# sharwarimarathe/GossipProtocol

Hardware: AMD Instinct MI355X
Metric: node-updates/sec (whole node) + achieved HBM GB/s %, imp3D push-sum 1e9 nodes (higher is better)
Workload: dtype f64; 1 GPU; push-sum rounds, Imp3D lattice, n=1000000000 (P=1000000000), steady state (all nodes active), seed 1; num_nodes=1000000000, population=1000000000, topology=Imp3D, algorithm=push-sum, parallelism=slab1, transport=none (one GPU), launcher=single process, activation_preroll_rounds=72

## Files before the change

### gossipprotocol_amd/csrc/gp_device.hpp

```cpp
#pragma once

#include <hip/hip_runtime.h>
#include <stdint.h>

#define GP_HD __host__ __device__ __forceinline__

namespace gp {

enum Topology : int { LINE = 0, FULL = 1, GRID3D = 2, IMP3D = 3 };
enum Algorithm : int { GOSSIP = 0, PUSHSUM = 1 };
enum Stream : uint32_t { S_TOPO = 0, S_START = 1, S_GOSSIP = 2, S_PUSHSUM = 3, S_INJECT = 4 };

constexpr uint8_t DIR_MASK = 7, DIR_NONE = 7, DIR_RANDOM = 6;
constexpr uint8_t B_ACTIVE = 8, B_CONV = 16;
constexpr int CNT_SHIFT = 5;
constexpr uint32_t GOSSIP_DONE = 11;

GP_HD uint32_t xor3(uint32_t a, uint32_t b, uint32_t k) {
#if defined(__HIP_DEVICE_COMPILE__)
    uint32_t r;
    asm("v_bitop3_b32 %0, %1, %2, %3 bitop3:0x96" : "=v"(r) : "v"(a), "v"(b), "s"(k));
    return r;
#else
    return a ^ b ^ k;
#endif
}

GP_HD void philox2(uint32_t node, uint32_t round, uint32_t stream, uint32_t k0, uint32_t k1,
                   uint32_t& x, uint32_t& y) {
    uint32_t c0 = node, c1 = round, c2 = stream, c3 = 0;
#if defined(__HIP_DEVICE_COMPILE__)
    asm volatile("" : "+s"(k0), "+s"(k1));
#endif
#pragma unroll
    for (int r = 0; r < 10; ++r) {
        if (r) {
            k0 += 0x9E3779B9u;
            k1 += 0xBB67AE85u;
        }
        const uint64_t p0 = (uint64_t)0xD2511F53u * c0;
        const uint64_t p1 = (uint64_t)0xCD9E8D57u * c2;
        const uint32_t n0 = xor3((uint32_t)(p1 >> 32), c1, k0);
        const uint32_t n2 = xor3((uint32_t)(p0 >> 32), c3, k1);
        c1 = (uint32_t)p1;
        c3 = (uint32_t)p0;
        c0 = n0;
        c2 = n2;
    }
    x = c0;
    y = c1;
}

template <int N>
GP_HD void philox2_batch(const uint32_t (&node)[N], uint32_t round, uint32_t stream, uint32_t k0, uint32_t k1,
                         uint32_t (&x)[N], uint32_t (&y)[N]) {
    uint32_t c0[N], c1[N], c2[N], c3[N];
#pragma unroll
    for (int i = 0; i < N; ++i) {
        c0[i] = node[i];
        c1[i] = round;
        c2[i] = stream;
        c3[i] = 0;
    }
#if defined(__HIP_DEVICE_COMPILE__)
    asm volatile("" : "+s"(k0), "+s"(k1));
#endif
#pragma unroll
    for (int r = 0; r < 10; ++r) {
        if (r) {
            k0 += 0x9E3779B9u;
            k1 += 0xBB67AE85u;
        }
#pragma unroll
        for (int i = 0; i < N; ++i) {
            const uint64_t p0 = (uint64_t)0xD2511F53u * c0[i];
            const uint64_t p1 = (uint64_t)0xCD9E8D57u * c2[i];
            const uint32_t n0 = xor3((uint32_t)(p1 >> 32), c1[i], k0);
            const uint32_t n2 = xor3((uint32_t)(p0 >> 32), c3[i], k1);
            c1[i] = (uint32_t)p1;
            c3[i] = (uint32_t)p0;
            c0[i] = n0;
            c2[i] = n2;
        }
    }
#pragma unroll
    for (int i = 0; i < N; ++i) {
        x[i] = c0[i];
        y[i] = c1[i];
    }
}

GP_HD uint32_t uniform_from(uint32_t x, uint32_t y, uint32_t m) {
    const uint64_t lo = (uint64_t)x * m;
    const uint64_t hi = (uint64_t)y * m + (lo >> 32);
    return (uint32_t)(hi >> 32);
}

GP_HD uint32_t uniform(uint32_t k0, uint32_t k1, uint32_t stream, uint32_t node, uint32_t round,
                       uint32_t m) {
    uint32_t x, y;
    philox2(node, round, stream, k0, k1, x, y);
    return uniform_from(x, y, m);
}

GP_HD bool ratio_moved(double s, double w, double s2, double w2) {
    const double a = s * w2;
    const double b = __builtin_fma(s2, w, -a);
    const double m = w * w2;
    if (m >= 0x1p-900 && (s == 0.0 || a >= 0x1p-900) && __builtin_fabs(b) > 0x1p-18 * m) return true;
    return __builtin_fabs(s2 / w2 - s / w) > 1e-10;
}

struct FastDiv {
    uint32_t d;
    uint32_t magic;
    uint32_t shift;
    uint32_t mode;
};

inline FastDiv make_fastdiv(uint32_t d) {
    FastDiv f{d, 0, 0, 0};
    if (d == 0) return f;
    const uint32_t l = 31u - (uint32_t)__builtin_clz(d);
    if ((d & (d - 1)) == 0) {
        f.shift = l;
        f.mode = 0;
        return f;
    }
    const uint64_t num = 1ull << (32 + l);
    uint32_t proposed = (uint32_t)(num / d);
    const uint32_t rem = (uint32_t)(num % d);
    const uint32_t e = d - rem;
    if (e < (1u << l)) {
        f.shift = l;
        f.mode = 1;
    } else {
        proposed += proposed;
        const uint32_t twice_rem = rem + rem;
        if (twice_rem >= d || twice_rem < rem) proposed += 1;
        f.shift = l;
        f.mode = 2;
    }
    f.magic = 1u + proposed;
    return f;
}

GP_HD uint32_t mulhi32(uint32_t a, uint32_t b) { return (uint32_t)(((uint64_t)a * b) >> 32); }

GP_HD uint32_t fastdiv(uint32_t n, const FastDiv& f) {
    if (f.mode == 0) return n >> f.shift;
    const uint32_t q = mulhi32(f.magic, n);
    if (f.mode == 1) return q >> f.shift;
    const uint32_t t = ((n - q) >> 1) + q;
    return t >> f.shift;
}

struct Geom {
    uint32_t P;
    uint32_t T;
    uint32_t g, g2;
    FastDiv div_g, div_g2;
};

template <int TOPO>
GP_HD uint32_t present_mask(uint32_t j, const Geom& G) {
    if (TOPO == LINE) return (j > 0 ? 1u : 0u) | (j + 1 < G.P ? 2u : 0u);
    const uint32_t x = fastdiv(j, G.div_g2);
    const uint32_t rem = j - x * G.g2;
    const uint32_t y = fastdiv(rem, G.div_g);
    const uint32_t z = rem - y * G.g;
    const uint32_t gm = G.g - 1;
    return (x > 0 ? 1u : 0u) | (x < gm ? 2u : 0u) | (y < gm ? 4u : 0u) | (y > 0 ? 8u : 0u) |
           (z < gm ? 16u : 0u) | (z > 0 ? 32u : 0u);
}

template <int TOPO>
GP_HD uint32_t nbr(uint32_t j, uint32_t d, const Geom& G) {
    if (TOPO == LINE) return d == 0 ? j - 1 : j + 1;
    switch (d) {
        case 0: return j - G.g2;
        case 1: return j + G.g2;
        case 2: return j + G.g;
        case 3: return j - G.g;
        case 4: return j + 1;
        default: return j - 1;
    }
}

GP_HD uint32_t popc6(uint32_t m) {
#if defined(__HIP_DEVICE_COMPILE__)
    return (uint32_t)__popc(m);
#else
    return (uint32_t)__builtin_popcount(m);
#endif
}

GP_HD uint32_t slot_to_dir(uint32_t mask, uint32_t k) {
#pragma unroll
    for (uint32_t d = 0; d < 6; ++d) {
        if (mask & (1u << d)) {
            if (k == 0) return d;
            --k;
        }
    }
    return DIR_RANDOM;
}

GP_HD uint32_t slot_to_dir_fast(uint32_t mask, uint32_t k) {
    if (mask == 63u) return k < 6u ? k : (uint32_t)DIR_RANDOM;
    return slot_to_dir(mask, k);
}

GP_HD uint32_t mask_xyz(uint32_t x, uint32_t y, uint32_t z, uint32_t gm) {
    return (x > 0 ? 1u : 0u) | (x < gm ? 2u : 0u) | (y < gm ? 4u : 0u) | (y > 0 ? 8u : 0u) | (z < gm ? 16u : 0u) |
           (z > 0 ? 32u : 0u);
}

GP_HD uint32_t full_target(uint32_t i, uint32_t k) { return k < i ? k : k + 1; }

}
```

### gossipprotocol_amd/csrc/gp_ps_tile.hip

```cpp
#include <type_traits>

#include "gp_tile.hpp"

namespace gp {
#ifdef GP_TILE_WIDE
namespace wide {
#endif

constexpr int PRIO = 1;

namespace {

template <bool REMOTE>
struct PsSlots {
    static constexpr bool SNDPF = !REMOTE;
    static constexpr int SLOTS = SNDPF ? TILE + TILE / 8 : TILE + TILE / 8 + TILE / 16;
    static constexpr int FU = (SLOTS + TPB - 1) / TPB;
};

template <bool REMOTE>
struct TileLdsP {
    static constexpr int SLOTS = PsSlots<REMOTE>::SLOTS, SLOT_FU = PsSlots<REMOTE>::FU;
    uint32_t rows[W_ROWS + DMA_SLACK];
    uint32_t xm[W_PLANE + DMA_SLACK];
    uint32_t xp[W_PLANE + DMA_SLACK];
    uint32_t ind[TILE / 8 + DMA_SLACK];
    unsigned long long bits[SLOT_FU * (TPB / 64) + 1];
    double2 msg[SLOTS];
    uint32_t out[TILE / 4];
    uint32_t red[2][TPB / 64];
    uint32_t qn[2];
    double2 zb[TPB / 64][NPT][2];
};

}

template <int TOPO, bool REMOTE>
__device__ __forceinline__ void ps_tiles(const RoundArgs& a, uint32_t r, TileLdsP<REMOTE>& L, uint32_t* snd,
                                         bool all_active, uint32_t& alerts, uint32_t& newly, bool& tiny) {
    const double2* __restrict__ swc = a.swc;
    double2* __restrict__ swn = a.swn;
    const uint64_t* __restrict__ rbc = a.rbc;
    const uint32_t* __restrict__ in_src = a.in_src;
    const bool packed = a.in_srcd != nullptr;
    const uint32_t* __restrict__ srcp = packed ? a.in_srcd : in_src;
    const Geom G = a.G;
    const uint32_t H = TOPO == LINE ? 1u : G.g;
    constexpr int FU = PsSlots<REMOTE>::FU;
    const uint32_t cap = min((uint32_t)PsSlots<REMOTE>::SLOTS, a.stage_cap);
    const uint32_t lane = threadIdx.x & 63u, wv = threadIdx.x >> 6;

    uint32_t pf_tile = 0xFFFFFFFFu, pf_lo = 0, pf_hi = 0;
    uint32_t snd_tile = 0xFFFFFFFFu, snd_off = 0;
    constexpr bool SNDPF = PsSlots<REMOTE>::SNDPF;
    uint32_t raw[FU];
#pragma unroll
    for (int m = 0; m < FU; ++m) raw[m] = 0u;
    TileWalk tw(a);
    const bool dyn = tw.mode == 3;
    uint32_t it = 0;
    if (dyn) {
        if (blockIdx.x == 0 && threadIdx.x < 8) a.tq_next[threadIdx.x * TQ_STRIDE] = 0u;
        if (threadIdx.x == 0) L.qn[0] = atomicAdd(tw.qc, 1u);
        __syncthreads();
        tw.t = __builtin_amdgcn_readfirstlane(L.qn[0]);
        ++it;
    }
    for (uint32_t victim = 0;;) {
    while (tw.t < tw.end) {
        uint32_t ti;
        uint32_t claim = 0;
        if (dyn && threadIdx.x == 0) claim = atomicAdd(tw.qc, 1u);
        if (!tw.tile(ti)) {
            if (dyn) {
                if (threadIdx.x == 0) L.qn[it & 1] = claim;
                __syncthreads();
                tw.t = __builtin_amdgcn_readfirstlane(L.qn[it & 1]);
                ++it;
            } else {
                tw.t += tw.step;
            }
            continue;
        }
        const uint32_t T = (a.lo / TILE + ti) * TILE;
        const uint32_t j0 = max(a.lo, T);
        const uint32_t j1 = min(a.lo + a.nloc, T + TILE);
        const bool have_pf = pf_tile == ti;
        uint32_t e_lo = 0, e_hi = 0;
        if (TOPO == IMP3D) {
            if (have_pf) {
                e_lo = pf_lo;
                e_hi = pf_hi;
            } else {
                e_lo = ld_const(a.in_off + j0);
                e_hi = ld_const(a.in_off + j1);
            }
        }
        const uint32_t cnt = e_hi - e_lo;
        const bool staged = cnt <= cap;
        if (TOPO == IMP3D && !dyn) {
            TileWalk nw = tw;
            nw.t += nw.step;
            uint32_t nti;
            pf_tile = 0xFFFFFFFFu;
            if (nw.t < nw.end && nw.tile(nti)) {
                const uint32_t nT = (a.lo / TILE + nti) * TILE;
                pf_lo = ld_const(a.in_off + max(a.lo, nT));
                pf_hi = ld_const(a.in_off + min(a.lo + a.nloc, nT + TILE));
                pf_tile = nti;
            }
        }
        if constexpr (TOPO == IMP3D) {
            if (staged) {
                if (SNDPF && snd_tile == ti) {
                    uint32_t ts = threadIdx.x;
                    asm volatile("" : "+v"(ts));
#pragma unroll
                    for (int m = 0; m < FU; ++m) {
                        const uint32_t q = ts + m * TPB;
                        raw[m] = q < cnt ? snd[snd_off + q] : 0u;
                    }
                } else {
#pragma unroll
                    for (int m = 0; m < FU; ++m) {
                        const uint32_t q = threadIdx.x + m * TPB;
                        raw[m] = q < cnt ? __builtin_nontemporal_load(srcp + e_lo + q) : 0u;
                    }
                }
                uint32_t rkv[REMOTE ? FU : 1];
                if constexpr (REMOTE) {
#pragma unroll
                    for (int m = 0; m < FU; ++m) {
                        const uint32_t q = threadIdx.x + m * TPB;
                        rkv[m] = q < cnt ? __builtin_nontemporal_load(a.rk + e_lo + q) : 0u;
                    }
                }
                uint32_t isrc[FU];
                bool sent[FU], pick[FU];
#pragma unroll
                for (int m = 0; m < FU; ++m) isrc[m] = packed ? raw[m] & 0x3FFFFFFFu : raw[m];
                if (all_active) {
                    constexpr int F0 = FU < NPT ? FU : NPT;
                    uint32_t x[FU], y[FU];
                    {
                        uint32_t n0[F0], x0[F0], y0[F0];
#pragma unroll
                        for (int m = 0; m < F0; ++m) n0[m] = isrc[m];
                        philox2_batch<F0>(n0, r, S_PUSHSUM, a.k0, a.k1, x0, y0);
#pragma unroll
                        for (int m = 0; m < F0; ++m) {
                            x[m] = x0[m];
                            y[m] = y0[m];
                        }
                    }
#pragma unroll
                    for (int m = F0; m < FU; ++m) {
                        x[m] = y[m] = 0u;
                        if (cnt > (uint32_t)(m * TPB) + (__builtin_amdgcn_readfirstlane(threadIdx.x) & ~63u)) {
                            uint32_t n1[1] = {isrc[m]}, x1[1], y1[1];
                            philox2_batch<1>(n1, r, S_PUSHSUM, a.k0, a.k1, x1, y1);
                            x[m] = x1[0];
                            y[m] = y1[0];
                        }
                    }
#pragma unroll
                    for (int m = 0; m < FU; ++m) {
                        const uint32_t q = threadIdx.x + m * TPB;
                        const uint32_t di = packed ? (raw[m] >> 30) + 4u : popc6(present_mask<IMP3D>(isrc[m], G)) + 1u;
                        sent[m] = pick[m] = q < cnt && uniform_from(x[m], y[m], di) == di - 1u;
                    }
                } else {
                    uint32_t x[FU], y[FU];
                    philox2_batch<FU>(isrc, r, S_PUSHSUM, a.k0, a.k1, x, y);
                    bool lpick[FU];
#pragma unroll
                    for (int m = 0; m < FU; ++m) {
                        const uint32_t q = threadIdx.x + m * TPB;
                        const uint32_t i = isrc[m];
                        const uint32_t di = packed ? (raw[m] >> 30) + 4u : popc6(present_mask<IMP3D>(i, G)) + 1u;
                        pick[m] = q < cnt && uniform_from(x[m], y[m], di) == di - 1u;
                        lpick[m] = pick[m] && (!REMOTE || i - a.lo < a.nloc);
                    }
                    unsigned long long wbits[FU];
#pragma unroll
                    for (int m = 0; m < FU; ++m) wbits[m] = rbc[lpick[m] ? (isrc[m] >> 6) - (a.lo >> 6) : 0u];
#pragma unroll
                    for (int m = 0; m < FU; ++m) asm volatile("" : "+v"(wbits[m])::"memory");
#pragma unroll
                    for (int m = 0; m < FU; ++m) wbits[m] = lpick[m] ? wbits[m] : 0ull;
#pragma unroll
                    for (int m = 0; m < FU; ++m) sent[m] = (wbits[m] >> (isrc[m] & 63)) & 1ull;
                }
                uint32_t ridx[REMOTE ? FU : 1];
                if constexpr (REMOTE) {
                    uint2 hm[FU];
                    uint32_t hb[FU];
#pragma unroll
                    for (int m = 0; m < FU; ++m) {
                        const bool cand = pick[m] && isrc[m] - a.lo >= a.nloc;
                        const XHdr* hp = a.xhdr + (cand ? rkv[m] >> 6 : 0u);
                        hm[m] = *reinterpret_cast<const uint2*>(&hp->mask);
                        hb[m] = hp->base;
                    }
#pragma unroll
                    for (int m = 0; m < FU; ++m) asm volatile("" : "+v"(hm[m].x), "+v"(hm[m].y), "+v"(hb[m])::"memory");
#pragma unroll
                    for (int m = 0; m < FU; ++m) {
                        ridx[m] = 0u;
                        if (pick[m] && isrc[m] - a.lo >= a.nloc) {
                            const unsigned long long mk = ((unsigned long long)hm[m].y << 32) | hm[m].x;
                            const uint32_t bit = rkv[m] & 63u;
                            sent[m] = (mk >> bit) & 1ull;
                            ridx[m] = min(hb[m] + (uint32_t)__popcll(mk & ((1ull << bit) - 1ull)), a.xnv - 1u);
                        }
                    }
                }
                __builtin_amdgcn_s_setprio(PRIO);
#pragma unroll
                for (int m = 0; m < FU; ++m) {
                    const unsigned long long bal = __ballot(sent[m]);
                    if (lane == 0) L.bits[m * (TPB / 64) + wv] = bal;
                    if (sent[m]) {
                        const double2* src;
                        if constexpr (REMOTE) {
                            uint32_t xi = ridx[m];
                            asm volatile("" : "+v"(xi));
                            src = isrc[m] - a.lo >= a.nloc ? a.xvals + xi : swc + isrc[m];
                        } else {
                            src = swc + isrc[m];
                        }
                        __builtin_amdgcn_global_load_lds((gvoid_t*)src, (lvoid_t*)(L.msg + (m * TPB + wv * 64)), 16,
                                                         0, DMA_ONCE);
                    }
                }
                if (threadIdx.x == 0) {
                    unsigned long long z = 0ull;
                    asm volatile("" : "+v"(z));
                    L.bits[FU * (TPB / 64)] = z;
                }
            }
        }
        double2 own[NPT];
        const uint32_t b_rows = dma_stage_bytes(L.rows, a.nbc, (int64_t)j0 - H, (int64_t)j1 + H, a.ext_lo, a.ext_hi);
        uint32_t b_xm = 0, b_xp = 0;
        if (TOPO != LINE) {
            b_xm = dma_stage_bytes(L.xm, a.nbc, (int64_t)j0 - G.g2, (int64_t)j1 - G.g2, a.ext_lo, a.ext_hi);
            b_xp = dma_stage_bytes(L.xp, a.nbc, (int64_t)j0 + G.g2, (int64_t)j1 + G.g2, a.ext_lo, a.ext_hi);
        }
        {
            uint32_t zt = threadIdx.x;
            asm volatile("" : "+v"(zt));
            const uint32_t zl = zt & 63u, zw = zt >> 6;
            if (zl < 2u * NPT) {
                int64_t jn = (int64_t)T + (int64_t)((zl >> 1) * TPB + zw * 64u) + ((zl & 1u) ? 64 : -1);
                if (jn < (int64_t)a.ext_lo) jn = a.ext_lo;
                if (jn > (int64_t)a.ext_hi) jn = a.ext_hi;
                __builtin_amdgcn_global_load_lds((gvoid_t*)(swc + jn), (lvoid_t*)&L.zb[zw][0][0], 16, 0, 0);
            }
        }
        if (TOPO == IMP3D) {
            const uint8_t* ip = a.ind4 + T / 2;
            asm volatile("" : "+s"(ip));
            uint32_t nt = threadIdx.x;
            asm volatile("" : "+v"(nt));
            if (nt < (uint32_t)(TILE / 32))
                __builtin_amdgcn_global_load_lds((gvoid_t*)(ip + nt * 16u), (lvoid_t*)L.ind, 16, 0, DMA_ONCE);
        }
        if (dyn && threadIdx.x == 0) L.qn[it & 1] = claim;
        __builtin_amdgcn_s_setprio(0);
        __syncthreads();
        uint32_t cinc = 0;
        bool wide = false;
        if (TOPO == IMP3D) {
            const uint2 w2 = reinterpret_cast<const uint2*>(L.ind)[lane];
            auto nsum = [](uint32_t w) { return (((w & 0x0F0F0F0Fu) + ((w >> 4) & 0x0F0F0F0Fu)) * 0x01010101u) >> 24; };
            auto has15 = [](uint32_t w) { return (w & (w >> 1) & (w >> 2) & (w >> 3) & 0x11111111u) != 0u; };
            uint32_t incl = nsum(w2.x) + nsum(w2.y);
            wide = __ballot(has15(w2.x) || has15(w2.y)) != 0ull;
#pragma unroll
            for (int o = 1; o < 64; o <<= 1) {
                const uint32_t t = __shfl_up(incl, o, 64);
                if (lane >= (uint32_t)o) incl += t;
            }
            const uint32_t ex = __shfl_up(incl, 1, 64);
            cinc = lane == 0 ? 0u : ex;
        }
        uint32_t t_next = tw.t + tw.step;
        if (dyn) {
            t_next = __builtin_amdgcn_readfirstlane(L.qn[it & 1]);
            ++it;
            if (TOPO == IMP3D) {
                TileWalk nw = tw;
                nw.t = t_next;
                uint32_t nti;
                pf_tile = 0xFFFFFFFFu;
                if (nw.t < nw.end && nw.tile(nti)) {
                    const uint32_t nT = (a.lo / TILE + nti) * TILE;
                    pf_lo = ld_const(a.in_off + max(a.lo, nT));
                    pf_hi = ld_const(a.in_off + min(a.lo + a.nloc, nT + TILE));
                    pf_tile = nti;
                }
            }
        }

        bool full = j0 == T && j1 == T + TILE && (TOPO != IMP3D || (staged && !wide));
#ifdef GP_EXPERIMENTS
        if (a.no_full) full = false;
#endif
        auto tile_body = [&](auto full_c, auto shadow_c) {
        constexpr bool FULL = decltype(full_c)::value;
        constexpr bool SHADOW = decltype(shadow_c)::value;
        uint32_t tid = threadIdx.x;
        asm volatile("" : "+v"(tid));
        const uint32_t lane = tid & 63u, wv = tid >> 6;
        uint32_t pend[(NPT + 1) / 2];
#pragma unroll
        for (int k = 0; k < (NPT + 1) / 2; ++k) pend[k] = 0u;
        {
            const uint32_t wbase = __builtin_amdgcn_readfirstlane(tid & ~63u);
            uint32_t wcx = 0, wcy = 0, wcz = 0;
            if (TOPO != LINE) {
                const uint32_t jw = T + wbase;
                wcx = fastdiv(jw, G.div_g2);
                const uint32_t rem = jw - wcx * G.g2;
                wcy = fastdiv(rem, G.div_g);
                wcz = rem - wcy * G.g;
            }
            constexpr uint32_t NDG = TOPO == LINE ? 0u : 4u;
            auto decide = [&](const int k, uint32_t& gst, uint32_t& epre) {
                epre = 0u;
                uint32_t edeg = 0u;
                if (TOPO == IMP3D) {
                    const uint32_t jl = k * TPB + tid;
                    const uint32_t d = (lds_byte(L.ind, jl >> 1) >> ((jl & 1u) * 4u)) & 15u;
                    uint32_t ex = mbcnt64(__ballot(d & 1u)) + 2u * mbcnt64(__ballot(d & 2u));
                    if (__ballot(d >= 4u)) ex += 4u * mbcnt64(__ballot(d & 4u)) + 8u * mbcnt64(__ballot(d & 8u));
                    const int wvu = __builtin_amdgcn_readfirstlane((int)wv);
                    epre = (uint32_t)__builtin_amdgcn_readlane((int)cinc, 16 * k + 4 * wvu) + ex;
                    edeg = d;
                }
                const uint32_t j = T + k * TPB + tid;
                if (TOPO != LINE && k > 0) {
                    wcz += TPB;
                    if (wcz >= G.g) {
                        const uint32_t q = fastdiv(wcz, G.div_g);
                        wcz -= q * G.g;
                        wcy += q;
                        if (wcy >= G.g) {
                            const uint32_t q2 = fastdiv(wcy, G.div_g);
                            wcy -= q2 * G.g;
                            wcx += q2;
                        }
                    }
                }
                const uint32_t jr = j - b_rows;
                const uint32_t gbv = lds_byte(L.rows, jr);
                uint32_t mask;
                if (TOPO == LINE) {
                    mask = present_mask<TOPO>(j, G);
                } else {
                    const uint32_t gm = G.g - 1u;
                    const bool interior = wcz >= 1u && wcz + 64u < gm && wcy >= 1u && wcy < gm && wcx >= 1u && wcx < gm;
                    mask = interior ? 63u : present_mask<TOPO>(j, G);
                }
                uint32_t from = 0;
                if (TOPO == LINE) {
                    from |= ((mask & 1u) && (lds_byte(L.rows, (mask & 1u) ? jr - 1 : jr) & DIR_MASK) == 1u) ? 1u : 0u;
                    from |= ((mask & 2u) && (lds_byte(L.rows, (mask & 2u) ? jr + 1 : jr) & DIR_MASK) == 0u) ? 2u : 0u;
                } else {
                    const uint32_t bxm = lds_byte(L.xm, (mask & 1u) ? j - G.g2 - b_xm : 0u);
                    const uint32_t bxp = lds_byte(L.xp, (mask & 2u) ? j + G.g2 - b_xp : 0u);
                    const uint32_t byp = lds_byte(L.rows, (mask & 4u) ? jr + G.g : jr);
                    const uint32_t bym = lds_byte(L.rows, (mask & 8u) ? jr - G.g : jr);
                    uint32_t bzp, bzm;
                    if constexpr (FULL) {
                        const uint32_t be = lds_byte(L.rows, lane == 63u ? jr + 1u : max(jr, 1u) - 1u);
                        bzp = (uint32_t)__builtin_amdgcn_mov_dpp((int)gbv, 0x130, 0xF, 0xF, true);
                        bzm = (uint32_t)__builtin_amdgcn_mov_dpp((int)gbv, 0x138, 0xF, 0xF, true);
                        if (lane == 63u) bzp = be;
                        if (lane == 0u) bzm = be;
                    } else {
                        bzp = lds_byte(L.rows, (mask & 16u) ? jr + 1 : jr);
                        bzm = lds_byte(L.rows, (mask & 32u) ? jr - 1 : jr);
                    }
                    from =((bxm & DIR_MASK) == 1u ? 1u : 0u) | ((bxp & DIR_MASK) == 0u ? 2u : 0u) |
                           ((byp & DIR_MASK) == 3u ? 4u : 0u) | ((bym & DIR_MASK) == 2u ? 8u : 0u) |
                           ((bzp & DIR_MASK) == 5u ? 16u : 0u) | ((bzm & DIR_MASK) == 4u ? 32u : 0u);
                    from &= mask;
                }
                if (!FULL && !(j >= j0 && j < j1)) from = 0u;
                gst = gbv | (mask << 8) | (from << 14) | (edeg << 20);
            };
            constexpr bool AHEAD = SHADOW;
            uint32_t gst_n = 0u, epre_n = 0u;
            if (AHEAD) {
                __builtin_amdgcn_s_setprio(PRIO);
                decide(0, gst_n, epre_n);
            }
#pragma unroll
            for (int k = 0; k < NPT; ++k) {
                __builtin_amdgcn_s_setprio(PRIO);
                uint32_t gst, epre;
                if (AHEAD) {
                    gst = gst_n;
                    epre = epre_n;
                } else {
                    decide(k, gst, epre);
                }
                const uint32_t jl = k * TPB + tid;
                const uint32_t j = T + jl;
                double2 m[NDG > 0 ? NDG : 1];
                {
                    const uint32_t from = (gst >> 14) & 63u;
                    own[k] = swc[FULL ? j : min(max(j, j0), j1 - 1u)];
#pragma unroll
                    for (uint32_t d = 0; d < NDG; ++d)
                        m[d] = ld_sw(swc + ((from >> d) & 1u ? nbr<TOPO>(j, d, G) : a.ext_hi));
                }
                __builtin_amdgcn_s_setprio(0);
                if (SHADOW) __builtin_amdgcn_sched_barrier(0);
                {
                    const bool valid = FULL || (j >= j0 && j < j1);
                    uint32_t pwin = 0u, pqb = 0u;
                    if (TOPO == IMP3D && (FULL || (staged && !wide))) {
                        const uint32_t* bw = reinterpret_cast<const uint32_t*>(L.bits);
                        pqb = epre;
                        const uint32_t nd = gst >> 20;
                        pwin = __builtin_amdgcn_alignbit(bw[(pqb >> 5) + 1], bw[pqb >> 5], pqb & 31u) & ((1u << nd) - 1u);
                    }
                    if (SHADOW) {
                        uint32_t x, y;
                        philox2(j, r + 1, S_PUSHSUM, a.k0, a.k1, x, y);
                        const uint32_t mask = (gst >> 8) & 63u;
                        const uint32_t cand = slot_to_dir_fast(mask, uniform_from(x, y, popc6(mask) + (TOPO == IMP3D ? 1u : 0u)));
                        pend[k >> 1] |= cand << (16 * (k & 1));
                        if (AHEAD && k + 1 < NPT) decide(k + 1, gst_n, epre_n);
                        __builtin_amdgcn_sched_barrier(0);
                    }
                    double2 zP = make_double2(0.0, 0.0), zM = zP;
                    {
                        constexpr uint32_t dP = TOPO == LINE ? 1u : 4u, dM = TOPO == LINE ? 0u : 5u;
                        const uint32_t from = (gst >> 14) & 63u;
                        zP = dpp_double2<0x130>(own[k]);
                        zM = dpp_double2<0x138>(own[k]);
                        if (lane == 63u) zP = L.zb[wv][k][1];
                        if (lane == 0u) zM = L.zb[wv][k][0];
                        if (!((from >> dP) & 1u)) zP = make_double2(0.0, 0.0);
                        else if (!FULL && lane != 63u && j + 1u >= j1) zP = ld_sw(swc + j + 1);
                        if (!((from >> dM) & 1u)) zM = make_double2(0.0, 0.0);
                        else if (!FULL && lane != 0u && j <= j0) zM = ld_sw(swc + j - 1);
                    }
                    __builtin_amdgcn_s_waitcnt(vmcnt_enc(0));
                    if (valid) {
                        const uint32_t b = gst & 0xFFu, mask = (gst >> 8) & 63u, from = (gst >> 14) & 63u;
                        const uint32_t deg = popc6(mask) + (TOPO == IMP3D ? 1u : 0u);
                        bool active = (b & B_ACTIVE) != 0;
                        const double2 sv = own[k];

                        const bool halve = active && deg > 0;
                        const double hf = halve ? 0.5 : 1.0;
                        double acc_s = sv.x * hf;
                        double acc_w = sv.y * hf;
                        auto fold = [&](const double2 mi) {
                            acc_s = __builtin_fma(mi.x, 0.5, acc_s);
                            acc_w = __builtin_fma(mi.y, 0.5, acc_w);
                        };
                        tiny |= (sv.y < 0x1p-1020) | (sv.x != 0.0 && sv.x < 0x1p-1020);
                        bool recv = from != 0;
                        if (TOPO == LINE) {
                            fold(zM);
                            fold(zP);
                        } else {
#pragma unroll
                            for (uint32_t d = 0; d < NDG; ++d) fold(m[d]);
                            fold(zP);
                            fold(zM);
                        }
                        if (TOPO == IMP3D) {
                            uint32_t e_b = e_lo + epre, e_e = e_b + (gst >> 20);
                            if (!FULL && wide) {
                                e_b = a.in_off[j];
                                e_e = a.in_off[j + 1];
                            }
                            if (FULL || (staged && !wide)) {
                                uint32_t win = pwin;
                                while (win) {
                                    const uint32_t q = pqb + (uint32_t)__builtin_ctz(win);
                                    win &= win - 1u;
                                    fold(L.msg[q]);
                                    recv = true;
                                }
                            } else if (staged) {
                                const uint32_t* bw = reinterpret_cast<const uint32_t*>(L.bits);
                                const uint32_t qe = e_e - e_lo;
                                for (uint32_t q0 = e_b - e_lo; q0 < qe; q0 += 32u) {
                                    uint32_t win = __builtin_amdgcn_alignbit(bw[(q0 >> 5) + 1], bw[q0 >> 5], q0 & 31u);
                                    if (qe - q0 < 32u) win &= (1u << (qe - q0)) - 1u;
                                    while (win) {
                                        const uint32_t q = q0 + (uint32_t)__builtin_ctz(win);
                                        win &= win - 1u;
                                        fold(L.msg[q]);
                                        recv = true;
                                    }
                                }
                            } else {
                                for (uint32_t e = e_b; e < e_e; ++e) {
                                    const uint32_t i = in_src[e];
                                    bool sent;
                                    double2 mi = make_double2(0.0, 0.0);
                                    const bool rem = REMOTE && i - a.lo >= a.nloc;
                                    uint32_t xi = 0;
                                    if (rem) {
                                        const uint32_t k = a.rk[e];
                                        const XHdr h = a.xhdr[k >> 6];
                                        sent = (h.mask >> (k & 63u)) & 1ull;
                                        xi = min(h.base + (uint32_t)__popcll(h.mask & ((1ull << (k & 63u)) - 1ull)),
                                                 a.xnv - 1u);
                                    } else if (all_active) {
                                        const uint32_t di = popc6(present_mask<IMP3D>(i, G)) + 1u;
                                        sent = uniform(a.k0, a.k1, S_PUSHSUM, i, r, di) == di - 1u;
                                    } else {
                                        sent = (rbc[(i >> 6) - (a.lo >> 6)] >> (i & 63)) & 1ull;
                                    }
                                    if (sent) mi = rem ? a.xvals[xi] : ld_sw(swc + i);
                                    if (sent) {
                                        fold(mi);
                                        recv = true;
                                    }
                                }
                            }
                        }
                        uint32_t flags = b & (B_ACTIVE | B_CONV | (3u << CNT_SHIFT));
                        if (recv) {
                            if (!(b & B_CONV)) {
                                uint32_t cnt3 = (b >> CNT_SHIFT) & 3u;
                                cnt3 = ratio_moved(sv.x, sv.y, acc_s, acc_w) ? 0u : cnt3 + 1u;
                                flags = (flags & ~(3u << CNT_SHIFT)) | (cnt3 << CNT_SHIFT);
                                if (cnt3 == 3) {
                                    flags |= B_CONV;
                                    ++alerts;
                                }
                            }
                            if (!active) {
                                ++newly;
                                flags |= B_ACTIVE;
                                active = true;
                            }
                        }
                        if (SHADOW) {
                            pend[k >> 1] |= ((active && deg > 0 ? 0u : (uint32_t)DIR_NONE) | (flags & 0x78u)) << (16 * (k & 1));
                        } else {
                            pend[k >> 1] |= (mask | (active && deg > 0 ? 64u : 0u) | ((flags >> 3) << 7)) << (16 * (k & 1));
                        }
                        st_stream(swn + j, make_double2(acc_s, acc_w));
                    }
                }
                if (SNDPF && TOPO == IMP3D && k == 0) {
                    snd_tile = 0xFFFFFFFFu;
                    if (pf_tile != 0xFFFFFFFFu && pf_hi - pf_lo <= cap) {
                        snd_off = dma_stage_words(snd, srcp, pf_lo, pf_hi);
                        snd_tile = pf_tile;
                    }
                }
            }
        }
        {
            uint32_t node[NPT], x[NPT], y[NPT];
#pragma unroll
            for (int k = 0; k < NPT; ++k) node[k] = T + k * TPB + tid;
            if (!SHADOW) philox2_batch<NPT>(node, r + 1, S_PUSHSUM, a.k0, a.k1, x, y);
#pragma unroll
            for (int k = 0; k < NPT; ++k) {
                const uint32_t jl = k * TPB + tid;
                const bool valid = FULL || (node[k] >= j0 && node[k] < j1);
                const uint32_t pk = pend[k >> 1] >> (16 * (k & 1));
                uint32_t dir, nb;
                if (SHADOW) {
                    dir = pk & DIR_MASK;
                    nb = pk & 0x7Fu;
                } else {
                    const uint32_t mask = pk & 63u;
                    dir = DIR_NONE;
                    if (pk & 64u) dir = slot_to_dir_fast(mask, uniform_from(x[k], y[k], popc6(mask) + (TOPO == IMP3D ? 1u : 0u)));
                    nb = (((pk >> 7) & 15u) << 3) | dir;
                }
                if (valid) reinterpret_cast<uint8_t*>(L.out)[jl] = (uint8_t)nb;
                if (TOPO == IMP3D) {
                    const unsigned long long bits = __ballot(valid && dir == DIR_RANDOM);
                    if (lane == 0) {
                        const int64_t wi = (int64_t)((T + k * TPB + (tid & ~63u)) >> 6) - (int64_t)(a.lo >> 6);
                        if (wi >= 0) a.rbn[wi] = bits;
                    }
                }
            }
        }
        __syncthreads();
        for (uint32_t w = tid; w < (uint32_t)(TILE / 4); w += TPB) {
            const uint32_t jw = T + w * 4;
            if (FULL || (jw >= j0 && jw + 4 <= j1)) {
                st_stream(reinterpret_cast<uint32_t*>(a.nbn + T) + w, L.out[w]);
            } else {
                for (uint32_t b = 0; b < 4; ++b)
                    if (jw + b >= j0 && jw + b < j1) a.nbn[jw + b] = reinterpret_cast<const uint8_t*>(L.out)[w * 4 + b];
            }
        }
        };
#ifdef GP_EXPERIMENTS
        if (!a.slot_shadow) {
            if (full) tile_body(std::true_type{}, std::false_type{});
            else tile_body(std::false_type{}, std::false_type{});
        } else
#endif
        if (full) tile_body(std::true_type{}, std::true_type{});
        else tile_body(std::false_type{}, std::true_type{});
        tw.t = t_next;
    }
        if (!dyn || ++victim >= 8u) break;
        const uint32_t c = (blockIdx.x + victim) & 7u;
        tw.qc = a.tq + c * TQ_STRIDE;
        tw.wl = a.wt + a.wo[c];
        tw.end = a.wo[c + 1] - a.wo[c];
        if (threadIdx.x == 0) L.qn[it & 1] = atomicAdd(tw.qc, 1u);
        __syncthreads();
        tw.t = __builtin_amdgcn_readfirstlane(L.qn[it & 1]);
        ++it;
    }
}

__device__ __forceinline__ void block_counts(uint32_t (*red)[TPB / 64], uint32_t& x, uint32_t& y) {
    uint32_t tid = threadIdx.x;
    asm volatile("" : "+v"(tid));
    const uint32_t lane = tid & 63u, wv = tid >> 6;
#pragma unroll
    for (int o = 32; o > 0; o >>= 1) {
        x += __shfl_xor(x, o, 64);
        y += __shfl_xor(y, o, 64);
    }
    if (lane == 0) {
        red[0][wv] = x;
        red[1][wv] = y;
    }
    __syncthreads();
    if (threadIdx.x == 0) {
        x = 0;
        y = 0;
        for (int w = 0; w < TPB / 64; ++w) {
            x += red[0][w];
            y += red[1][w];
        }
    }
}

__device__ __forceinline__ void add_round_counts(Ctl* ctl, uint32_t x, uint32_t y) {
    unsigned long long d = 0;
    if (x) d += __hip_atomic_fetch_add(&ctl->round_alerts, (unsigned long long)x, __ATOMIC_RELAXED,
                                       __HIP_MEMORY_SCOPE_AGENT);
    if (y) d += __hip_atomic_fetch_add(&ctl->round_active, (unsigned long long)y, __ATOMIC_RELAXED,
                                       __HIP_MEMORY_SCOPE_AGENT);
    asm volatile("" ::"v"(d));
    __builtin_amdgcn_s_waitcnt(0);
}

template <int TOPO, bool REMOTE>
__global__ __launch_bounds__(TPB, GP_MINB) void k_ps_tile(RoundArgs a, uint32_t r) {
    __shared__ TileLdsP<REMOTE> L;
    __shared__ uint32_t snd[PsSlots<REMOTE>::SNDPF ? PsSlots<REMOTE>::SLOTS + DMA_SLACK : 1];
    Ctl* ctl = a.ctl;
    if (ld_agent(&ctl->done)) return;
    const bool all_active = ld_agent(&ctl->all_active) != 0;
    uint32_t alerts = 0, newly = 0;
    bool tiny = false;
    ps_tiles<TOPO, REMOTE>(a, r, L, snd, all_active, alerts, newly, tiny);
    if (__ballot(tiny) && (threadIdx.x & 63u) == 0) atomicOr(&ctl->tiny, 1u);
    block_counts(L.red, alerts, newly);
    if (threadIdx.x == 0) {
        if (a.fuse == 2) {
            block_done_close_sharded(ctl, a.G.P, a.G.T, r, alerts, newly);
        } else if (a.fuse) {
            add_round_counts(ctl, alerts, newly);
            block_done_close(ctl, a.G.P, a.G.T, r);
        } else {
            if (alerts) atomicAdd(&ctl->round_alerts, (unsigned long long)alerts);
            if (newly) atomicAdd(&ctl->round_active, (unsigned long long)newly);
        }
    }
}


using PsTileKernel = void (*)(RoundArgs, uint32_t);
static PsTileKernel ps_tile_kernel(int topo, bool remote) {
    if (topo == LINE) return k_ps_tile<LINE, false>;
    if (topo == GRID3D) return k_ps_tile<GRID3D, false>;
#ifndef GP_TILE_WIDE
    if (topo == IMP3D) return remote ? k_ps_tile<IMP3D, true> : k_ps_tile<IMP3D, false>;
#endif
    return nullptr;
}

int ps_tile_resident_blocks(int topo, bool remote, int device) {
    const PsTileKernel f = ps_tile_kernel(topo, remote);
    int per_cu = 0, cus = 0;
    if (!f) return 0;
    if (hipOccupancyMaxActiveBlocksPerMultiprocessor(&per_cu, reinterpret_cast<const void*>(f), TPB, 0) != hipSuccess)
        return 0;
    if (hipDeviceGetAttribute(&cus, hipDeviceAttributeMultiprocessorCount, device) != hipSuccess) return 0;
    return per_cu * cus;
}

hipError_t launch_ps_tile(const DevState& S, const RoundArgs& a, uint32_t round, int grid, hipStream_t st) {
    const PsTileKernel f = ps_tile_kernel(S.topo, S.rk != nullptr);
    if (!f || (S.topo == IMP3D && !S.ind4)) return hipErrorInvalidValue;
    hipLaunchKernelGGL(f, dim3(grid), dim3(TPB), 0, st, a, round);
    return hipGetLastError();
}

#ifdef GP_TILE_WIDE
}
#else
hipError_t launch_round_tile_region(const DevState& S, uint32_t round, uint32_t h, int grid, hipStream_t st) {
    if (S.alg != PUSHSUM || S.topo != IMP3D || !S.rk || !S.ind4 || !S.wtiles || S.tile_walk != 3 ||
        h >= S.rregions || (grid & 7))
        return hipErrorInvalidValue;
    RoundArgs a = make_round_args(S, round);
    for (int c = 0; c <= 8; ++c) a.wo[c] = S.woff[h][c];
    const uint64_t L = (uint64_t)round * S.rregions + h;
    a.tq = S.tq + (L & 1) * 8 * TQ_STRIDE;
    a.tq_next = S.tq + ((L + 1) & 1) * 8 * TQ_STRIDE;
    hipLaunchKernelGGL((k_ps_tile<IMP3D, true>), dim3(grid), dim3(TPB), 0, st, a, round);
    return hipGetLastError();
}
#endif
}
```

Before: 83.71 billion node-updates/s.

## Decode tile direction bytes four-per-lane with SWAR and redistribute via bpermute

For full interior tiles with four nodes per thread, each lane now reads one 32-bit word of direction bytes per neighbour plane and computes the six 'from' flags for four nodes at once using byte-parallel bit tricks. For Imp3D it also builds the per-node edge prefix offsets with a byte prefix sum plus DPP row scans. Each node's results are then fetched back to its owning lane with ds_bpermute. This is meant to replace per-node LDS byte loads and scalar decode in the decide step. It adds cross-lane permutes and more intricate index arithmetic, with risk of edge-case mistakes at tile borders.

```diff
diff --git a/gossipprotocol_amd/csrc/gp_device.hpp b/gossipprotocol_amd/csrc/gp_device.hpp
--- a/gossipprotocol_amd/csrc/gp_device.hpp
+++ b/gossipprotocol_amd/csrc/gp_device.hpp
@@ -216,6 +216,34 @@
            (z > 0 ? 32u : 0u);
 }
 
+
+GP_HD uint32_t byte_window(uint32_t lo, uint32_t hi, uint32_t ph) {
+#if defined(__HIP_DEVICE_COMPILE__)
+    return __builtin_amdgcn_alignbyte(hi, lo, ph);
+#else
+    return (uint32_t)((((uint64_t)hi << 32) | lo) >> (8u * (ph & 3u)));
+#endif
+}
+
+GP_HD uint32_t dir_ne4(uint32_t w, uint32_t d) {
+    return (((w ^ (d * 0x01010101u)) & 0x07070707u) + 0x07070707u) & 0x08080808u;
+}
+
+GP_HD uint32_t from4(const uint32_t (&ne)[6]) {
+    const uint32_t any = (ne[0] >> 3) | (ne[1] >> 2) | (ne[2] >> 1) | ne[3] | (ne[4] << 1) | (ne[5] << 2);
+    return ~any & 0x3F3F3F3Fu;
+}
+
+GP_HD uint32_t nibbles_to_bytes(uint32_t x) {
+    x = (x | (x << 8)) & 0x00FF00FFu;
+    return (x | (x << 4)) & 0x0F0F0F0Fu;
+}
+
+GP_HD uint32_t byte_prefix4(uint32_t b) {
+    b += b << 8;
+    return b + (b << 16);
+}
+
 GP_HD uint32_t full_target(uint32_t i, uint32_t k) { return k < i ? k : k + 1; }
 
 }
diff --git a/gossipprotocol_amd/csrc/gp_ps_tile.hip b/gossipprotocol_amd/csrc/gp_ps_tile.hip
--- a/gossipprotocol_amd/csrc/gp_ps_tile.hip
+++ b/gossipprotocol_amd/csrc/gp_ps_tile.hip
@@ -391,11 +391,87 @@
                 if (!FULL && !(j >= j0 && j < j1)) from = 0u;
                 gst = gbv | (mask << 8) | (from << 14) | (edeg << 20);
             };
+            constexpr bool PASS = FULL && TOPO != LINE && NPT == 4;
+            uint32_t pA = 0u, pF = 0u, pW[2] = {0u, 0u};
+            if constexpr (PASS) {
+                static_assert(!PASS || TPB * NPT == 64 * 4 * (TPB / 64), "a wave's slots are one word per lane");
+                const uint32_t jl4 = (lane >> 4) * TPB + wbase + 4u * (lane & 15u);
+                const uint32_t j4 = T + jl4;
+                auto window = [](const uint32_t* base, const int32_t o) {
+                    const int32_t wi = o >> 2;
+                    return byte_window(base[max(wi, 0)], base[max(wi + 1, 0)], (uint32_t)o & 3u);
+                };
+                const int32_t o = (int32_t)(j4 - b_rows);
+                const int32_t wi = o >> 2;
+                const uint32_t ph = (uint32_t)o & 3u;
+                const uint32_t w0 = L.rows[wi], w1 = L.rows[wi + 1], wp = L.rows[max(wi - 1, 0)];
+                pA = byte_window(w0, w1, ph);
+                const uint32_t wzp = byte_window(pA, byte_window(w1, 0u, ph), 1u);
+                const uint32_t wzm = byte_window(byte_window(wp, w0, ph), pA, 3u);
+                const uint32_t ne[6] = {dir_ne4(window(L.xm, (int32_t)(j4 - G.g2 - b_xm)), 1u),
+                                        dir_ne4(window(L.xp, (int32_t)(j4 + G.g2 - b_xp)), 0u),
+                                        dir_ne4(window(L.rows, o + (int32_t)G.g), 3u),
+                                        dir_ne4(window(L.rows, o - (int32_t)G.g), 2u),
+                                        dir_ne4(wzp, 5u),
+                                        dir_ne4(wzm, 4u)};
+                pF = from4(ne);
+                if (TOPO == IMP3D) {
+                    const uint32_t db = nibbles_to_bytes(reinterpret_cast<const uint16_t*>(L.ind)[jl4 >> 2]);
+                    const uint32_t incl = byte_prefix4(db);
+                    uint32_t run = incl >> 24;
+                    run += (uint32_t)__builtin_amdgcn_mov_dpp((int)run, 0x111, 0xF, 0xF, true);
+                    run += (uint32_t)__builtin_amdgcn_mov_dpp((int)run, 0x112, 0xF, 0xF, true);
+                    run += (uint32_t)__builtin_amdgcn_mov_dpp((int)run, 0x114, 0xF, 0xF, true);
+                    run += (uint32_t)__builtin_amdgcn_mov_dpp((int)run, 0x118, 0xF, 0xF, true);
+                    const uint32_t base = run - (incl >> 24);
+                    const uint32_t excl = incl << 8, b2 = base | (base << 16);
+                    pW[0] = (excl & 0x00FF00FFu) + b2 + ((db & 0x00FF00FFu) << 10);
+                    pW[1] = ((excl >> 8) & 0x00FF00FFu) + b2 + (((db >> 8) & 0x00FF00FFu) << 10);
+                }
+            }
+            auto fetch = [&](const int k, uint32_t& gst, uint32_t& epre) {
+                const int src = (int)((16u * k + (lane >> 2)) << 2);
+                const uint32_t sh = (lane & 3u) * 8u;
+                const uint32_t gbv = ((uint32_t)__builtin_amdgcn_ds_bpermute(src, (int)pA) >> sh) & 0xFFu;
+                uint32_t from = ((uint32_t)__builtin_amdgcn_ds_bpermute(src, (int)pF) >> sh) & 63u;
+                epre = 0u;
+                uint32_t edeg = 0u;
+                if (TOPO == IMP3D) {
+                    const uint32_t v0 = (uint32_t)__builtin_amdgcn_ds_bpermute(src, (int)pW[0]);
+                    const uint32_t v1 = (uint32_t)__builtin_amdgcn_ds_bpermute(src, (int)pW[1]);
+                    const uint32_t v = ((lane & 1u) ? v1 : v0) >> ((lane & 2u) * 8u);
+                    const int wvu = __builtin_amdgcn_readfirstlane((int)wv);
+                    epre = (uint32_t)__builtin_amdgcn_readlane((int)cinc, 16 * k + 4 * wvu) + (v & 0x3FFu);
+                    edeg = (v >> 10) & 15u;
+                }
+                if (k > 0) {
+                    wcz += TPB;
+                    if (wcz >= G.g) {
+                        const uint32_t q = fastdiv(wcz, G.div_g);
+                        wcz -= q * G.g;
+                        wcy += q;
+                        if (wcy >= G.g) {
+                            const uint32_t q2 = fastdiv(wcy, G.div_g);
+                            wcy -= q2 * G.g;
+                            wcx += q2;
+                        }
+                    }
+                }
+                const uint32_t gm = G.g - 1u;
+                const bool interior = wcz >= 1u && wcz + 64u < gm && wcy >= 1u && wcy < gm && wcx >= 1u && wcx < gm;
+                const uint32_t mask = interior ? 63u : present_mask<TOPO>(T + k * TPB + tid, G);
+                from &= mask;
+                gst = gbv | (mask << 8) | (from << 14) | (edeg << 20);
+            };
+            auto settle = [&](const int k, uint32_t& gst, uint32_t& epre) {
+                if constexpr (PASS) fetch(k, gst, epre);
+                else decide(k, gst, epre);
+            };
             constexpr bool AHEAD = SHADOW;
             uint32_t gst_n = 0u, epre_n = 0u;
             if (AHEAD) {
                 __builtin_amdgcn_s_setprio(PRIO);
-                decide(0, gst_n, epre_n);
+                settle(0, gst_n, epre_n);
             }
 #pragma unroll
             for (int k = 0; k < NPT; ++k) {
@@ -405,7 +481,7 @@
                     gst = gst_n;
                     epre = epre_n;
                 } else {
-                    decide(k, gst, epre);
+                    settle(k, gst, epre);
                 }
                 const uint32_t jl = k * TPB + tid;
                 const uint32_t j = T + jl;
@@ -434,7 +510,7 @@
                         const uint32_t mask = (gst >> 8) & 63u;
                         const uint32_t cand = slot_to_dir_fast(mask, uniform_from(x, y, popc6(mask) + (TOPO == IMP3D ? 1u : 0u)));
                         pend[k >> 1] |= cand << (16 * (k & 1));
-                        if (AHEAD && k + 1 < NPT) decide(k + 1, gst_n, epre_n);
+                        if (AHEAD && k + 1 < NPT) settle(k + 1, gst_n, epre_n);
                         __builtin_amdgcn_sched_barrier(0);
                     }
                     double2 zP = make_double2(0.0, 0.0), zM = zP;
```

After: 83.95 billion node-updates/s (median of 6 runs). No clear change (+0.3%).
